# rkhosrowshahi/MO-VAE

Measured on NVIDIA B200. Metric: aggregation_GBps, higher is better.
Workload: dtype f32

## Files before the change

### mo-vae_b200/csrc/aggregate.cu

```cuda
#include "recombine_device.cuh"
#include "solve_device.cuh"

namespace movae {

int fill_solve_params(int k, const movae_solve_spec* spec, SolveParams* out);
int check_solve_vectors(const SolveParams& p, const float* d_vec, const float* d_aux);

constexpr int kAggThreads = 256;
static_assert(kAggThreads == kGramThreads && kAggThreads == kRecThreads && kAggThreads == kSolveThreads, "one CTA shape");

struct AggArgs {
    const float* J;
    int64_t P, ldJ;
    unsigned char* ws;
    const float* vec;
    const float* aux;
    float* out;
    int accumulate;
    float* w_out;
    double* diag_out;
    double* G_out;
};

template <int K>
__device__ __forceinline__ void aggregate_solve_phase(const SolveParams& sp, const P2PArgs& px, const float* vec, const float* aux,
                                                      float* w_out, double* diag_out, double* G_out, const double* partials,
                                                      unsigned int* ticket, unsigned int* ready, unsigned int ready0,
                                                      unsigned long long* stamps, unsigned long long t_start) {
    __shared__ SolveSmem S;
    __shared__ double Gs[K * K];
    __shared__ unsigned long long seq_s;
    __shared__ int failed_s;
    const int tid = threadIdx.x;
    const unsigned long long t_in = global_timer_ns();
    gram_combine_partials<K>(partials, Gs);
    if (tid == 0) { *ticket = 0u; failed_s = 0; stamps[4] = global_timer_ns(); }
    if (px.world > 0) {
        XchgBuffer* own = px.peers[px.rank];
        if (tid == 0) seq_s = own->step + 1;
        __syncthreads();
        const unsigned long long seq = seq_s;
        const int par = (int)(seq & 1ull);
        if (tid < K * K) {
            const double v = Gs[tid];
            for (int r = 0; r < px.world; ++r) st_relaxed_sys_f64(&px.peers[r]->slots[par][px.rank][tid], v);
        }
        __threadfence_system();
        __syncthreads();
        if (tid < px.world) st_release_sys_u64(&px.peers[tid]->flags[par][px.rank], seq);
        if (tid == 0) own->step = seq;
        if (tid < px.world && !wait_flag_sys(&own->flags[par][tid], seq, kExchangeTimeoutNs)) failed_s = 1;
        __syncthreads();
        if (tid < K * K) {
            double g = 0.0;
            for (int r = 0; r < px.world; ++r) g += ld_relaxed_sys_f64(&own->slots[par][r][tid]);
            Gs[tid] = g;
        }
        __syncthreads();
    }
    if (tid == 0) stamps[5] = global_timer_ns();
    if (tid < MK * MK) {
        const int i = tid / MK, j = tid % MK;
        S.G[i][j] = (i < K && j < K) ? Gs[i * K + j] : 0.0;
    }
    if (G_out && tid < K * K) G_out[tid] = Gs[tid];
    __syncthreads();
    solve_block<K>(sp, S, vec, aux, failed_s != 0, tid);
    if (tid < K) {
        w_out[tid] = S.w[tid];
        if (sp.comfort) w_out[K + tid] = S.w2[tid];
    }
    __syncthreads();
    if (tid == 0) {
        stamps[0] = t_start;
        stamps[1] = t_in;
        stamps[2] = global_timer_ns();
        __threadfence();
        st_release_gpu_u32(ready, ready0 + 1u);
    }
    solve_diagnostics(sp, S, tid);
    __syncthreads();
    if (tid < MOVAE_DIAG_DOUBLES && diag_out) diag_out[tid] = S.dg[tid];
}

__device__ __forceinline__ void aggregate_wait_ready(const unsigned int* ready, unsigned int ready0) {
    if (threadIdx.x == 0) {
        const unsigned long long t0 = global_timer_ns();
        while (ld_acquire_gpu_u32(ready) == ready0) {
            __nanosleep(40);
            if (global_timer_ns() - t0 > 2ull * kExchangeTimeoutNs) break;
        }
    }
    __syncthreads();
}

template <int K, int U1, int U2, bool VEC, int MINB>
__global__ void __launch_bounds__(kAggThreads, MINB)
aggregate_kernel(AggArgs a, SolveParams sp, P2PArgs px) {
    constexpr int NACC = GramAcc<K>::N;
    const int tid = threadIdx.x;
    unsigned int* ticket = reinterpret_cast<unsigned int*>(a.ws);
    unsigned int* done = reinterpret_cast<unsigned int*>(a.ws + 4);
    unsigned int* ready = reinterpret_cast<unsigned int*>(a.ws + 128);
    unsigned long long* stamps = reinterpret_cast<unsigned long long*>(a.ws + 192);
    double* partials = reinterpret_cast<double*>(a.ws + kGramHeaderBytes);

    __shared__ unsigned int ready0;
    __shared__ unsigned long long t_start;
    __shared__ double red[kGramThreads / 32][NACC];
    __shared__ int is_last;
    if (tid == 0) {
        ready0 = ld_acquire_gpu_u32(ready);
        t_start = global_timer_ns();
    }

    double acc64[NACC];
#pragma unroll
    for (int i = 0; i < NACC; ++i) acc64[i] = 0.0;
    gram_stream_tiles<K, U1, VEC>(a.J, a.P, a.ldJ, acc64);
    const bool last = gram_cta_partial_and_ticket<K>(acc64, partials, ticket, red, &is_last);

    if (last) aggregate_solve_phase<K>(sp, px, a.vec, a.aux, a.w_out, a.diag_out, a.G_out, partials, ticket, ready, ready0, stamps, t_start);
    if (a.out == nullptr) return;

    recombine_tiles<K, U2, VEC>(a.J, a.P, a.ldJ, a.w_out, a.out, a.accumulate, [&] {
        if (!last) aggregate_wait_ready(ready, ready0);
    });
    __syncthreads();
    if (tid == 0) {
        if (atomicAdd(done, 1u) == gridDim.x - 1) {
            stamps[3] = global_timer_ns();
            *done = 0u;
        }
    }
}

template <int K, int U1, int U2, bool VEC, int MINB>
static int launch_aggregate(const AggArgs& a, const SolveParams& sp, const P2PArgs& px, cudaStream_t st) {
    auto kern = aggregate_kernel<K, U1, U2, VEC, MINB>;
    static thread_local int occ_dev = -1, occ = 0;
    int dev = 0;
    MOVAE_CUDA_TRY(cudaGetDevice(&dev));
    if (occ_dev != dev) {
        MOVAE_CUDA_TRY(cudaOccupancyMaxActiveBlocksPerMultiprocessor(&occ, kern, kAggThreads, 0));
        if (occ < 1) occ = 1;
        occ_dev = dev;
    }
    const int sms = sm_count();
    MOVAE_REQUIRE(sms > 0, MOVAE_ERR_CUDA, "CUDA device query failed (no GPU?)");
    const int64_t n_items = a.P / (VEC ? 4 : 1);
    const int64_t tile_items = (int64_t)kAggThreads * (U1 > U2 ? U1 : U2);
    int64_t n_tiles = (n_items + tile_items - 1) / tile_items;
    if (n_tiles < 1) n_tiles = 1;
    int64_t grid = (int64_t)sms * occ;
    if (grid > n_tiles) grid = n_tiles;
    if (grid > kGramMaxBlocks) grid = kGramMaxBlocks;
    AggArgs a_ = a;
    SolveParams sp_ = sp;
    P2PArgs px_ = px;
    void* params[] = {&a_, &sp_, &px_};
    MOVAE_CUDA_TRY(cudaLaunchCooperativeKernel(reinterpret_cast<const void*>(kern), dim3((unsigned)grid), dim3(kAggThreads), params, 0, st));
    return MOVAE_OK;
}

template <int K>
static int dispatch_aggregate(const AggArgs& a, const SolveParams& sp, const P2PArgs& px, cudaStream_t st) {
    const bool vec = (reinterpret_cast<uintptr_t>(a.J) % 16 == 0) && (a.out == nullptr || reinterpret_cast<uintptr_t>(a.out) % 16 == 0) &&
                     (a.ldJ % 4 == 0 || K == 1);
    if (vec) {
        if constexpr (K <= 2) return launch_aggregate<K, 8, 4, true, 2>(a, sp, px, st);
        else if constexpr (K == 3) return launch_aggregate<K, 4, 4, true, 2>(a, sp, px, st);
        else if constexpr (K == 4) return launch_aggregate<K, 4, 2, true, 2>(a, sp, px, st);
        else return launch_aggregate<K, 2, 2, true, 1>(a, sp, px, st);
    } else {
        if constexpr (K <= 4) return launch_aggregate<K, 8, 8, false, 2>(a, sp, px, st);
        else return launch_aggregate<K, 4, 4, false, 1>(a, sp, px, st);
    }
}

struct SegArgs {
    movae_jac_segments segs;
    unsigned char* ws;
    const float* vec;
    const float* aux;
    float* out;
    int accumulate;
    float* w_out;
    double* diag_out;
    double* G_out;
};

template <int K, int U, int MINB>
__global__ void __launch_bounds__(kAggThreads, MINB)
aggregate_seg_kernel(const __grid_constant__ SegArgs a, SolveParams sp, P2PArgs px) {
    constexpr int NACC = GramAcc<K>::N;
    constexpr int kTile = kAggThreads * U;
    const int tid = threadIdx.x;
    unsigned int* ticket = reinterpret_cast<unsigned int*>(a.ws);
    unsigned int* done = reinterpret_cast<unsigned int*>(a.ws + 4);
    unsigned int* ready = reinterpret_cast<unsigned int*>(a.ws + 128);
    unsigned long long* stamps = reinterpret_cast<unsigned long long*>(a.ws + 192);
    double* partials = reinterpret_cast<double*>(a.ws + kGramHeaderBytes);
    const int n_seg = a.segs.n_segments;

    __shared__ unsigned int ready0;
    __shared__ unsigned long long t_start;
    __shared__ double red[kGramThreads / 32][NACC];
    __shared__ int is_last;
    __shared__ int tile_start[MOVAE_MAX_SEGMENTS + 1];
    if (tid == 0) {
        ready0 = ld_acquire_gpu_u32(ready);
        t_start = global_timer_ns();
        int acc = 0;
        for (int s = 0; s < n_seg; ++s) {
            tile_start[s] = acc;
            acc += (int)(((a.segs.n[s] >> 2) + kTile - 1) / kTile);
        }
        tile_start[n_seg] = acc;
    }
    __syncthreads();
    const int n_tiles = tile_start[n_seg];
    auto segment_of = [&](int v) { int s = 0; while (v >= tile_start[s + 1]) ++s; return s; };

    double acc64[NACC];
#pragma unroll
    for (int i = 0; i < NACC; ++i) acc64[i] = 0.0;
    for (int v = blockIdx.x; v < n_tiles; v += gridDim.x) {
        const int s = segment_of(v);
        const int64_t n_items = a.segs.n[s] >> 2;
        const int64_t base = (int64_t)(v - tile_start[s]) * kTile + tid;
        float4 x[K][U];
#pragma unroll
        for (int i = 0; i < K; ++i) {
            const float4* row = reinterpret_cast<const float4*>(a.segs.rows[s][i]);
#pragma unroll
            for (int u = 0; u < U; ++u) {
                const int64_t idx = base + u * kAggThreads;
                x[i][u] = idx < n_items ? ld_stream_f4(row + idx) : make_float4(0.f, 0.f, 0.f, 0.f);
            }
        }
        float acc[NACC];
#pragma unroll
        for (int q = 0; q < NACC; ++q) acc[q] = 0.f;
#pragma unroll
        for (int u = 0; u < U; ++u) {
            float c[K];
#pragma unroll
            for (int i = 0; i < K; ++i) c[i] = x[i][u].x;
            gram_fma<K>(acc, c);
#pragma unroll
            for (int i = 0; i < K; ++i) c[i] = x[i][u].y;
            gram_fma<K>(acc, c);
#pragma unroll
            for (int i = 0; i < K; ++i) c[i] = x[i][u].z;
            gram_fma<K>(acc, c);
#pragma unroll
            for (int i = 0; i < K; ++i) c[i] = x[i][u].w;
            gram_fma<K>(acc, c);
        }
#pragma unroll
        for (int q = 0; q < NACC; ++q) acc64[q] += (double)acc[q];
    }
    if (blockIdx.x == 0 && tid < 4 * n_seg) {
        const int s = tid >> 2, e = tid & 3;
        const int64_t c0 = a.segs.n[s] & ~(int64_t)3;
        if (c0 + e < a.segs.n[s]) {
            float c[K];
            float acc[NACC];
#pragma unroll
            for (int q = 0; q < NACC; ++q) acc[q] = 0.f;
#pragma unroll
            for (int i = 0; i < K; ++i) c[i] = a.segs.rows[s][i][c0 + e];
            gram_fma<K>(acc, c);
#pragma unroll
            for (int q = 0; q < NACC; ++q) acc64[q] += (double)acc[q];
        }
    }
    const bool last = gram_cta_partial_and_ticket<K>(acc64, partials, ticket, red, &is_last);

    if (last) aggregate_solve_phase<K>(sp, px, a.vec, a.aux, a.w_out, a.diag_out, a.G_out, partials, ticket, ready, ready0, stamps, t_start);
    if (a.out == nullptr) return;

    float w[K];
    bool have_w = false;
    for (int v = n_tiles - 1 - (int)blockIdx.x; v >= 0; v -= gridDim.x) {
        const int s = segment_of(v);
        const int64_t n_items = a.segs.n[s] >> 2;
        const int64_t base = (int64_t)(v - tile_start[s]) * kTile + tid;
        float4 x[K][U];
#pragma unroll
        for (int i = 0; i < K; ++i) {
            const float4* row = reinterpret_cast<const float4*>(a.segs.rows[s][i]);
#pragma unroll
            for (int u = 0; u < U; ++u) {
                const int64_t idx = base + u * kAggThreads;
                x[i][u] = idx < n_items ? ld_stream_f4(row + idx) : make_float4(0.f, 0.f, 0.f, 0.f);
            }
        }
        if (!have_w) {
            if (!last) aggregate_wait_ready(ready, ready0);
#pragma unroll
            for (int i = 0; i < K; ++i) w[i] = __ldcg(a.w_out + i);
            have_w = true;
        }
        float4* dst = reinterpret_cast<float4*>(a.out + a.segs.out_off[s]);
#pragma unroll
        for (int u = 0; u < U; ++u) {
            const int64_t idx = base + u * kAggThreads;
            if (idx >= n_items) continue;
            float4 o;
            o.x = w[0] * x[0][u].x; o.y = w[0] * x[0][u].y; o.z = w[0] * x[0][u].z; o.w = w[0] * x[0][u].w;
#pragma unroll
            for (int i = 1; i < K; ++i) {
                o.x = fmaf(w[i], x[i][u].x, o.x); o.y = fmaf(w[i], x[i][u].y, o.y);
                o.z = fmaf(w[i], x[i][u].z, o.z); o.w = fmaf(w[i], x[i][u].w, o.w);
            }
            if (a.accumulate) {
                const float4 old = dst[idx];
                o.x += old.x; o.y += old.y; o.z += old.z; o.w += old.w;
            }
            st_stream_f4(dst + idx, o);
        }
    }
    if (!have_w) {
        if (!last) aggregate_wait_ready(ready, ready0);
#pragma unroll
        for (int i = 0; i < K; ++i) w[i] = __ldcg(a.w_out + i);
    }
    if (blockIdx.x == 0 && tid < 4 * n_seg) {
        const int s = tid >> 2, e = tid & 3;
        const int64_t c = (a.segs.n[s] & ~(int64_t)3) + e;
        if (c < a.segs.n[s]) {
            float o = w[0] * a.segs.rows[s][0][c];
#pragma unroll
            for (int i = 1; i < K; ++i) o = fmaf(w[i], a.segs.rows[s][i][c], o);
            float* dst = a.out + a.segs.out_off[s] + c;
            *dst = a.accumulate ? *dst + o : o;
        }
    }
    __syncthreads();
    if (tid == 0) {
        if (atomicAdd(done, 1u) == gridDim.x - 1) {
            stamps[3] = global_timer_ns();
            *done = 0u;
        }
    }
}

template <int K, int U, int MINB>
static int launch_aggregate_seg(const SegArgs& a, const SolveParams& sp, const P2PArgs& px, cudaStream_t st) {
    auto kern = aggregate_seg_kernel<K, U, MINB>;
    static thread_local int occ_dev = -1, occ = 0;
    int dev = 0;
    MOVAE_CUDA_TRY(cudaGetDevice(&dev));
    if (occ_dev != dev) {
        MOVAE_CUDA_TRY(cudaOccupancyMaxActiveBlocksPerMultiprocessor(&occ, kern, kAggThreads, 0));
        if (occ < 1) occ = 1;
        occ_dev = dev;
    }
    const int sms = sm_count();
    MOVAE_REQUIRE(sms > 0, MOVAE_ERR_CUDA, "CUDA device query failed (no GPU?)");
    int64_t n_tiles = 0;
    for (int s = 0; s < a.segs.n_segments; ++s) n_tiles += ((a.segs.n[s] >> 2) + kAggThreads * U - 1) / (kAggThreads * U);
    if (n_tiles < 1) n_tiles = 1;
    int64_t grid = (int64_t)sms * occ;
    if (grid > n_tiles) grid = n_tiles;
    if (grid > kGramMaxBlocks) grid = kGramMaxBlocks;
    SegArgs a_ = a;
    SolveParams sp_ = sp;
    P2PArgs px_ = px;
    void* params[] = {&a_, &sp_, &px_};
    MOVAE_CUDA_TRY(cudaLaunchCooperativeKernel(reinterpret_cast<const void*>(kern), dim3((unsigned)grid), dim3(kAggThreads), params, 0, st));
    return MOVAE_OK;
}

}

extern "C" {

int movae_aggregate_f32(const float* d_J, int k, int64_t P, int64_t ldJ, const movae_solve_spec* spec, const float* d_vec,
                        const float* d_aux, float* d_grad, int accumulate, float* d_w, double* d_diag, double* d_G, void* d_ws,
                        size_t ws_bytes, const movae_p2p_ctx* ctx, void* stream) {
    using namespace movae;
    SolveParams sp;
    int rc = fill_solve_params(k, spec, &sp);
    if (rc != MOVAE_OK) return rc;
    rc = check_solve_vectors(sp, d_vec, d_aux);
    if (rc != MOVAE_OK) return rc;
    MOVAE_REQUIRE(P >= 0 && ldJ >= P, MOVAE_ERR_INVALID, "aggregate: need 0 <= P <= ldJ (P=%lld ldJ=%lld)", (long long)P, (long long)ldJ);
    MOVAE_REQUIRE(d_w != nullptr && (d_J != nullptr || P == 0), MOVAE_ERR_INVALID, "aggregate: null pointer");
    MOVAE_REQUIRE(d_ws != nullptr && ws_bytes >= movae_gram_workspace_bytes(k), MOVAE_ERR_WORKSPACE,
                  "aggregate: workspace too small (%zu < %zu)", ws_bytes, movae_gram_workspace_bytes(k));
    MOVAE_REQUIRE(reinterpret_cast<uintptr_t>(d_ws) % 8 == 0, MOVAE_ERR_WORKSPACE, "aggregate: workspace must be 8-byte aligned");
    P2PArgs px = p2p_disabled();
    if (ctx != nullptr) {
        rc = make_p2p_args(ctx, &px);
        if (rc != MOVAE_OK) return rc;
    }
    AggArgs a;
    a.J = d_J;
    a.P = P;
    a.ldJ = ldJ;
    a.ws = static_cast<unsigned char*>(d_ws);
    a.vec = d_vec;
    a.aux = d_aux;
    a.out = d_grad;
    a.accumulate = accumulate;
    a.w_out = d_w;
    a.diag_out = d_diag;
    a.G_out = d_G;
    cudaStream_t st = static_cast<cudaStream_t>(stream);
    switch (k) {
        case 1: return dispatch_aggregate<1>(a, sp, px, st);
        case 2: return dispatch_aggregate<2>(a, sp, px, st);
        case 3: return dispatch_aggregate<3>(a, sp, px, st);
        case 4: return dispatch_aggregate<4>(a, sp, px, st);
        case 5: return dispatch_aggregate<5>(a, sp, px, st);
        case 6: return dispatch_aggregate<6>(a, sp, px, st);
        case 7: return dispatch_aggregate<7>(a, sp, px, st);
        default: return dispatch_aggregate<8>(a, sp, px, st);
    }
}

int movae_aggregate_segments_f32(const movae_jac_segments* segs, const movae_solve_spec* spec, const float* d_vec,
                                 const float* d_aux, float* d_grad, int accumulate, float* d_w, double* d_diag, double* d_G,
                                 void* d_ws, size_t ws_bytes, const movae_p2p_ctx* ctx, void* stream) {
    using namespace movae;
    MOVAE_REQUIRE(segs != nullptr, MOVAE_ERR_INVALID, "aggregate_segments: null segment table");
    const int k = segs->k;
    SolveParams sp;
    int rc = fill_solve_params(k, spec, &sp);
    if (rc != MOVAE_OK) return rc;
    rc = check_solve_vectors(sp, d_vec, d_aux);
    if (rc != MOVAE_OK) return rc;
    MOVAE_REQUIRE(segs->n_segments >= 1 && segs->n_segments <= MOVAE_MAX_SEGMENTS, MOVAE_ERR_UNSUPPORTED,
                  "aggregate_segments: %d segments outside 1..%d", segs->n_segments, MOVAE_MAX_SEGMENTS);
    MOVAE_REQUIRE(d_w != nullptr, MOVAE_ERR_INVALID, "aggregate_segments: null pointer");
    MOVAE_REQUIRE(d_grad == nullptr || reinterpret_cast<uintptr_t>(d_grad) % 16 == 0, MOVAE_ERR_INVALID,
                  "aggregate_segments: the gradient buffer must be 16-byte aligned");
    for (int s = 0; s < segs->n_segments; ++s) {
        MOVAE_REQUIRE(segs->n[s] >= 0 && segs->out_off[s] >= 0 && segs->out_off[s] % 4 == 0, MOVAE_ERR_INVALID,
                      "aggregate_segments: segment %d needs n >= 0 and an output offset that is a multiple of 4", s);
        for (int i = 0; i < k; ++i)
            MOVAE_REQUIRE(segs->rows[s][i] != nullptr && reinterpret_cast<uintptr_t>(segs->rows[s][i]) % 16 == 0, MOVAE_ERR_INVALID,
                          "aggregate_segments: row %d of segment %d must be a 16-byte aligned device pointer", i, s);
    }
    MOVAE_REQUIRE(d_ws != nullptr && ws_bytes >= movae_gram_workspace_bytes(k), MOVAE_ERR_WORKSPACE,
                  "aggregate_segments: workspace too small (%zu < %zu)", ws_bytes, movae_gram_workspace_bytes(k));
    P2PArgs px = p2p_disabled();
    if (ctx != nullptr) {
        rc = make_p2p_args(ctx, &px);
        if (rc != MOVAE_OK) return rc;
    }
    SegArgs a;
    a.segs = *segs;
    a.ws = static_cast<unsigned char*>(d_ws);
    a.vec = d_vec;
    a.aux = d_aux;
    a.out = d_grad;
    a.accumulate = accumulate;
    a.w_out = d_w;
    a.diag_out = d_diag;
    a.G_out = d_G;
    cudaStream_t st = static_cast<cudaStream_t>(stream);
    switch (k) {
        case 1: return launch_aggregate_seg<1, 4, 2>(a, sp, px, st);
        case 2: return launch_aggregate_seg<2, 4, 2>(a, sp, px, st);
        case 3: return launch_aggregate_seg<3, 4, 2>(a, sp, px, st);
        case 4: return launch_aggregate_seg<4, 2, 2>(a, sp, px, st);
        case 5: return launch_aggregate_seg<5, 2, 1>(a, sp, px, st);
        case 6: return launch_aggregate_seg<6, 2, 1>(a, sp, px, st);
        case 7: return launch_aggregate_seg<7, 2, 1>(a, sp, px, st);
        default: return launch_aggregate_seg<8, 2, 1>(a, sp, px, st);
    }
}

int movae_aggregate_timestamps(const void* d_ws, uint64_t h_stamps[6], void* stream) {
    using namespace movae;
    MOVAE_REQUIRE(d_ws != nullptr && h_stamps != nullptr, MOVAE_ERR_INVALID, "aggregate_timestamps: null pointer");
    cudaStream_t st = static_cast<cudaStream_t>(stream);
    MOVAE_CUDA_TRY(cudaMemcpyAsync(h_stamps, static_cast<const unsigned char*>(d_ws) + 192, 6 * sizeof(uint64_t), cudaMemcpyDeviceToHost, st));
    MOVAE_CUDA_TRY(cudaStreamSynchronize(st));
    return MOVAE_OK;
}

}
```

### mo-vae_b200/csrc/common.cuh

```cuda
#pragma once
#include <cuda_runtime.h>
#include <stdint.h>
#include <stdio.h>
#include <string.h>

#include "../../include/movae_b200.h"

namespace movae {

void set_error(const char* fmt, ...);
int fail_cuda(cudaError_t e, const char* what);
int sm_count();

#define MOVAE_CUDA_TRY(expr)                                        \
    do {                                                            \
        cudaError_t _e = (expr);                                    \
        if (_e != cudaSuccess) return ::movae::fail_cuda(_e, #expr); \
    } while (0)

#define MOVAE_REQUIRE(cond, code, ...)          \
    do {                                        \
        if (!(cond)) {                          \
            ::movae::set_error(__VA_ARGS__);    \
            return (code);                      \
        }                                       \
    } while (0)

__device__ __forceinline__ float4 ld_stream_f4(const float4* p) {
    float4 v;
    asm volatile("ld.global.nc.L1::no_allocate.v4.f32 {%0,%1,%2,%3}, [%4];"
                 : "=f"(v.x), "=f"(v.y), "=f"(v.z), "=f"(v.w)
                 : "l"(p));
    return v;
}
__device__ __forceinline__ float ld_stream_f1(const float* p) {
    float v;
    asm volatile("ld.global.nc.L1::no_allocate.f32 %0, [%1];" : "=f"(v) : "l"(p));
    return v;
}
__device__ __forceinline__ void st_stream_f4(float4* p, float4 v) {
    asm volatile("st.global.cs.v4.f32 [%0], {%1,%2,%3,%4};" ::"l"(p), "f"(v.x), "f"(v.y), "f"(v.z), "f"(v.w)
                 : "memory");
}

struct XchgBuffer {
    double slots[2][MOVAE_MAX_WORLD][MOVAE_MAX_K * MOVAE_MAX_K];
    unsigned long long flags[2][MOVAE_MAX_WORLD];
    unsigned long long bar_flags[MOVAE_MAX_WORLD];
    unsigned long long step;
    unsigned long long bar_epoch;
};
struct P2PArgs {
    int rank, world;
    XchgBuffer* peers[MOVAE_MAX_WORLD];
};
__host__ __device__ inline P2PArgs p2p_disabled() {
    P2PArgs a;
    a.rank = 0;
    a.world = 0;
    for (int i = 0; i < MOVAE_MAX_WORLD; ++i) a.peers[i] = nullptr;
    return a;
}
int make_p2p_args(const movae_p2p_ctx* ctx, P2PArgs* out);

__device__ __forceinline__ void st_release_sys_u64(unsigned long long* p, unsigned long long v) {
    asm volatile("st.release.sys.global.u64 [%0], %1;" ::"l"(p), "l"(v) : "memory");
}
__device__ __forceinline__ unsigned long long ld_acquire_sys_u64(const unsigned long long* p) {
    unsigned long long v;
    asm volatile("ld.acquire.sys.global.u64 %0, [%1];" : "=l"(v) : "l"(p) : "memory");
    return v;
}
__device__ __forceinline__ double ld_relaxed_sys_f64(const double* p) {
    double v;
    asm volatile("ld.relaxed.sys.global.f64 %0, [%1];" : "=d"(v) : "l"(p) : "memory");
    return v;
}

__device__ __forceinline__ void st_relaxed_sys_f64(double* p, double v) {
    asm volatile("st.relaxed.sys.global.f64 [%0], %1;" ::"l"(p), "d"(v) : "memory");
}
__device__ __forceinline__ void st_release_gpu_u32(unsigned int* p, unsigned int v) {
    asm volatile("st.release.gpu.global.u32 [%0], %1;" ::"l"(p), "r"(v) : "memory");
}
__device__ __forceinline__ unsigned int ld_acquire_gpu_u32(const unsigned int* p) {
    unsigned int v;
    asm volatile("ld.acquire.gpu.global.u32 %0, [%1];" : "=r"(v) : "l"(p) : "memory");
    return v;
}
__device__ __forceinline__ unsigned long long global_timer_ns() {
    unsigned long long t;
    asm volatile("mov.u64 %0, %%globaltimer;" : "=l"(t));
    return t;
}
__device__ __forceinline__ bool wait_flag_sys(const unsigned long long* flag, unsigned long long want,
                                              unsigned long long timeout_ns) {
    if (ld_acquire_sys_u64(flag) >= want) return true;
    const unsigned long long t0 = global_timer_ns();
    while (ld_acquire_sys_u64(flag) < want) {
        if (global_timer_ns() - t0 > timeout_ns) return false;
    }
    return true;
}
constexpr unsigned long long kExchangeTimeoutNs = 20ull * 1000ull * 1000ull * 1000ull;

__device__ __forceinline__ double warp_sum(double v) {
#pragma unroll
    for (int o = 16; o > 0; o >>= 1) v += __shfl_xor_sync(0xffffffffu, v, o);
    return v;
}

}
```

### mo-vae_b200/csrc/gram_device.cuh

```cuda
#pragma once
#include "common.cuh"

namespace movae {

constexpr int kGramThreads = 256;
constexpr int kGramMaxBlocks = 2048;
constexpr int kGramHeaderBytes = 256;
constexpr int kGramChain = 64;

template <int K>
struct GramAcc {
    static constexpr int N = K * (K + 1) / 2;
};

template <int K>
__device__ __forceinline__ void gram_fma(float (&acc)[GramAcc<K>::N], const float (&x)[K]) {
    int a = 0;
#pragma unroll
    for (int i = 0; i < K; ++i)
#pragma unroll
        for (int j = i; j < K; ++j) { acc[a] = fmaf(x[i], x[j], acc[a]); ++a; }
}

struct RRSchedule {
    int64_t rounds;
    int64_t rem_lo, rem_hi;
};
__device__ __forceinline__ RRSchedule rr_schedule(int64_t n_items, int64_t tile_items, int64_t b, int64_t g) {
    RRSchedule s;
    s.rounds = (n_items / tile_items) / g;
    const int64_t r0 = s.rounds * g * tile_items;
    const int64_t m = (((n_items - r0) + g - 1) / g + 7) & ~(int64_t)7;
    s.rem_lo = r0 + b * m < n_items ? r0 + b * m : n_items;
    s.rem_hi = s.rem_lo + m < n_items ? s.rem_lo + m : n_items;
    return s;
}

template <int K, int U, bool VEC>
__device__ __forceinline__ void gram_tile(const float* __restrict__ J, int64_t ldJ, int64_t t0, int64_t hi, bool full,
                                          float (&acc)[GramAcc<K>::N]) {
    const int64_t base = t0 + threadIdx.x;
    if constexpr (VEC) {
        float4 v[K][U];
        if (full) {
#pragma unroll
            for (int i = 0; i < K; ++i)
#pragma unroll
                for (int u = 0; u < U; ++u)
                    v[i][u] = ld_stream_f4(reinterpret_cast<const float4*>(J + i * ldJ) + base + u * kGramThreads);
        } else {
#pragma unroll
            for (int i = 0; i < K; ++i)
#pragma unroll
                for (int u = 0; u < U; ++u) {
                    const int64_t idx = base + u * kGramThreads;
                    v[i][u] = idx < hi ? ld_stream_f4(reinterpret_cast<const float4*>(J + i * ldJ) + idx)
                                       : make_float4(0.f, 0.f, 0.f, 0.f);
                }
        }
#pragma unroll
        for (int u = 0; u < U; ++u) {
            float x[K];
#pragma unroll
            for (int i = 0; i < K; ++i) x[i] = v[i][u].x;
            gram_fma<K>(acc, x);
#pragma unroll
            for (int i = 0; i < K; ++i) x[i] = v[i][u].y;
            gram_fma<K>(acc, x);
#pragma unroll
            for (int i = 0; i < K; ++i) x[i] = v[i][u].z;
            gram_fma<K>(acc, x);
#pragma unroll
            for (int i = 0; i < K; ++i) x[i] = v[i][u].w;
            gram_fma<K>(acc, x);
        }
    } else {
        float v[K][U];
#pragma unroll
        for (int i = 0; i < K; ++i)
#pragma unroll
            for (int u = 0; u < U; ++u) {
                const int64_t idx = base + u * kGramThreads;
                v[i][u] = idx < hi ? ld_stream_f1(J + i * ldJ + idx) : 0.f;
            }
#pragma unroll
        for (int u = 0; u < U; ++u) {
            float x[K];
#pragma unroll
            for (int i = 0; i < K; ++i) x[i] = v[i][u];
            gram_fma<K>(acc, x);
        }
    }
}

template <int K, int U, bool VEC>
__device__ __forceinline__ void gram_stream_tiles(const float* __restrict__ J, int64_t P, int64_t ldJ,
                                                  double (&acc64)[GramAcc<K>::N]) {
    constexpr int NACC = GramAcc<K>::N;
    constexpr int W = VEC ? 4 : 1;
    constexpr int FLUSH = kGramChain / (W * U) > 0 ? kGramChain / (W * U) : 1;
    const int tid = threadIdx.x;
    const int64_t n_items = P / W;
    constexpr int64_t tile_items = (int64_t)kGramThreads * U;
    const RRSchedule sch = rr_schedule(n_items, tile_items, blockIdx.x, gridDim.x);

    int64_t r = 0;
    while (r < sch.rounds) {
        float acc[NACC];
#pragma unroll
        for (int a = 0; a < NACC; ++a) acc[a] = 0.f;
#pragma unroll 1
        for (int f = 0; f < FLUSH && r < sch.rounds; ++f, ++r) {
            const int64_t t0 = (r * gridDim.x + blockIdx.x) * tile_items;
            gram_tile<K, U, VEC>(J, ldJ, t0, t0 + tile_items, true, acc);
        }
#pragma unroll
        for (int a = 0; a < NACC; ++a) acc64[a] += (double)acc[a];
    }
    if (sch.rem_hi > sch.rem_lo) {
        float acc[NACC];
#pragma unroll
        for (int a = 0; a < NACC; ++a) acc[a] = 0.f;
        gram_tile<K, U, VEC>(J, ldJ, sch.rem_lo, sch.rem_hi, false, acc);
#pragma unroll
        for (int a = 0; a < NACC; ++a) acc64[a] += (double)acc[a];
    }

    if (VEC && blockIdx.x == 0 && tid < (int)(P - n_items * W)) {
        float x[K];
        float acc[NACC];
#pragma unroll
        for (int a = 0; a < NACC; ++a) acc[a] = 0.f;
#pragma unroll
        for (int i = 0; i < K; ++i) x[i] = J[i * ldJ + n_items * W + tid];
        gram_fma<K>(acc, x);
#pragma unroll
        for (int a = 0; a < NACC; ++a) acc64[a] += (double)acc[a];
    }
}

template <int K>
__device__ __forceinline__ bool gram_cta_partial_and_ticket(const double (&acc64)[GramAcc<K>::N], double* __restrict__ partials,
                                                            unsigned int* __restrict__ counter,
                                                            double (*red)[GramAcc<K>::N], int* is_last_smem) {
    constexpr int NACC = GramAcc<K>::N;
    const int tid = threadIdx.x, warp = tid >> 5, lane = tid & 31;
#pragma unroll
    for (int a = 0; a < NACC; ++a) {
        const double s = warp_sum(acc64[a]);
        if (lane == 0) red[warp][a] = s;
    }
    __syncthreads();
    if (tid < NACC) {
        double s = 0.0;
#pragma unroll
        for (int w = 0; w < kGramThreads / 32; ++w) s += red[w][tid];
        partials[(int64_t)blockIdx.x * NACC + tid] = s;
    }
    __threadfence();
    __syncthreads();
    if (tid == 0) *is_last_smem = (atomicAdd(counter, 1u) == gridDim.x - 1);
    __syncthreads();
    return *is_last_smem != 0;
}

template <int K>
__device__ __forceinline__ void gram_combine_partials(const double* __restrict__ partials, double* __restrict__ Gs) {
    constexpr int NACC = GramAcc<K>::N;
    const int tid = threadIdx.x, warp = tid >> 5, lane = tid & 31;
    __threadfence();
    for (int a = warp; a < NACC; a += kGramThreads / 32) {
        double s0 = 0.0, s1 = 0.0, s2 = 0.0, s3 = 0.0;
        const int g = (int)gridDim.x;
        for (int b = lane; b < g; b += 128) {
            const double v0 = __ldcg(&partials[(int64_t)b * NACC + a]);
            const double v1 = b + 32 < g ? __ldcg(&partials[(int64_t)(b + 32) * NACC + a]) : 0.0;
            const double v2 = b + 64 < g ? __ldcg(&partials[(int64_t)(b + 64) * NACC + a]) : 0.0;
            const double v3 = b + 96 < g ? __ldcg(&partials[(int64_t)(b + 96) * NACC + a]) : 0.0;
            s0 += v0; s1 += v1; s2 += v2; s3 += v3;
        }
        double s = (s0 + s1) + (s2 + s3);
        s = warp_sum(s);
        if (lane == 0) {
            int i = 0, rem = a;
            while (rem >= K - i) { rem -= K - i; ++i; }
            const int j = i + rem;
            Gs[i * K + j] = s;
            Gs[j * K + i] = s;
        }
    }
    __syncthreads();
}

}
```

### mo-vae_b200/csrc/recombine_device.cuh

```cuda
#pragma once
#include <type_traits>

#include "gram_device.cuh"

namespace movae {

constexpr int kRecThreads = 256;

template <int K, int U, bool VEC>
struct RecTile {
    using T = typename std::conditional<VEC, float4, float>::type;
    T v[K][U];
};

template <int K, int U, bool VEC>
__device__ __forceinline__ void rec_load_tile(RecTile<K, U, VEC>& r, const float* __restrict__ J, int64_t ldJ, int64_t base,
                                              int64_t lo, int64_t hi, bool full) {
#pragma unroll
    for (int i = 0; i < K; ++i)
#pragma unroll
        for (int u = 0; u < U; ++u) {
            const int64_t idx = base + u * kRecThreads;
            if constexpr (VEC)
                r.v[i][u] = (full || (idx >= lo && idx < hi)) ? ld_stream_f4(reinterpret_cast<const float4*>(J + i * ldJ) + idx)
                                                    : make_float4(0.f, 0.f, 0.f, 0.f);
            else
                r.v[i][u] = (full || (idx >= lo && idx < hi)) ? ld_stream_f1(J + i * ldJ + idx) : 0.f;
        }
}

template <int K, int U, bool VEC>
__device__ __forceinline__ void rec_store_tile(const RecTile<K, U, VEC>& r, const float (&w)[K], float* __restrict__ out,
                                               int64_t base, int64_t lo, int64_t hi, bool full, int accumulate) {
#pragma unroll
    for (int u = 0; u < U; ++u) {
        const int64_t idx = base + u * kRecThreads;
        if (!full && (idx < lo || idx >= hi)) continue;
        if constexpr (VEC) {
            float4 o;
            o.x = w[0] * r.v[0][u].x; o.y = w[0] * r.v[0][u].y; o.z = w[0] * r.v[0][u].z; o.w = w[0] * r.v[0][u].w;
#pragma unroll
            for (int i = 1; i < K; ++i) {
                o.x = fmaf(w[i], r.v[i][u].x, o.x); o.y = fmaf(w[i], r.v[i][u].y, o.y);
                o.z = fmaf(w[i], r.v[i][u].z, o.z); o.w = fmaf(w[i], r.v[i][u].w, o.w);
            }
            float4* dst = reinterpret_cast<float4*>(out) + idx;
            if (accumulate) {
                const float4 old = *dst;
                o.x += old.x; o.y += old.y; o.z += old.z; o.w += old.w;
            }
            st_stream_f4(dst, o);
        } else {
            float o = w[0] * r.v[0][u];
#pragma unroll
            for (int i = 1; i < K; ++i) o = fmaf(w[i], r.v[i][u], o);
            if (accumulate) o += out[idx];
            out[idx] = o;
        }
    }
}

template <int K, int U, bool VEC, class Ready>
__device__ __forceinline__ void recombine_tiles(const float* __restrict__ J, int64_t P, int64_t ldJ, const float* w_dev,
                                                float* __restrict__ out, int accumulate, Ready ready) {
    constexpr int W = VEC ? 4 : 1;
    const int tid = threadIdx.x;
    const int64_t n_items = P / W;
    constexpr int64_t tile_items = (int64_t)kRecThreads * U;
    const RRSchedule sch = rr_schedule(n_items, tile_items, blockIdx.x, gridDim.x);
    const bool has_rem = sch.rem_hi > sch.rem_lo;
    const int64_t n_steps = sch.rounds + (has_rem ? 1 : 0);
    auto t0_of = [&](int64_t i) -> int64_t {
        if (has_rem) { if (i == 0) return sch.rem_lo; --i; }
        return ((sch.rounds - 1 - i) * gridDim.x + blockIdx.x) * tile_items;
    };
    auto hi_of = [&](int64_t i, int64_t t0) -> int64_t { return (has_rem && i == 0) ? sch.rem_hi : t0 + tile_items; };
    auto full_of = [&](int64_t i) -> bool { return !(has_rem && i == 0); };

    RecTile<K, U, VEC> ra, rb;
    int64_t i = 0;
    int64_t ta = 0, tb = 0;
    if (n_steps > 0) { ta = t0_of(0); rec_load_tile<K, U, VEC>(ra, J, ldJ, ta + tid, ta, hi_of(0, ta), full_of(0)); }
    ready();
    float w[K];
#pragma unroll
    for (int q = 0; q < K; ++q) w[q] = __ldcg(w_dev + q);
    while (i < n_steps) {
        const bool has_b = i + 1 < n_steps;
        if (has_b) { tb = t0_of(i + 1); rec_load_tile<K, U, VEC>(rb, J, ldJ, tb + tid, tb, hi_of(i + 1, tb), full_of(i + 1)); }
        rec_store_tile<K, U, VEC>(ra, w, out, ta + tid, ta, hi_of(i, ta), full_of(i), accumulate);
        if (!has_b) break;
        if (i + 2 < n_steps) { ta = t0_of(i + 2); rec_load_tile<K, U, VEC>(ra, J, ldJ, ta + tid, ta, hi_of(i + 2, ta), full_of(i + 2)); }
        rec_store_tile<K, U, VEC>(rb, w, out, tb + tid, tb, hi_of(i + 1, tb), full_of(i + 1), accumulate);
        i += 2;
    }
    if (VEC && blockIdx.x == 0 && tid < (int)(P - n_items * W)) {
        const int64_t c = n_items * W + tid;
        float o = w[0] * J[c];
#pragma unroll
        for (int q = 1; q < K; ++q) o = fmaf(w[q], J[q * ldJ + c], o);
        if (accumulate) o += out[c];
        out[c] = o;
    }
}

}
```

Before: 6364.

## Pin tail of J in L2 with evict_last for reuse by recombine pass

The gram pass now loads the last rounds of J, sized to about two thirds of L2, with an evict_last cache policy. The recombine pass walks tiles in reverse order, so it can hit those lines in L2 instead of re-reading DRAM, and it demotes each consumed line back to evict_normal. This cuts DRAM traffic for the second read of J. It adds createpolicy and applypriority instructions, and the pinned data can crowd out other cached lines.

```diff
diff --git a/mo-vae_b200/csrc/aggregate.cu b/mo-vae_b200/csrc/aggregate.cu
--- a/mo-vae_b200/csrc/aggregate.cu
+++ b/mo-vae_b200/csrc/aggregate.cu
@@ -20,7 +20,10 @@
     float* w_out;
     double* diag_out;
     double* G_out;
+    int64_t keep_lo;
 };
+
+constexpr int64_t kL2KeepNum = 2, kL2KeepDen = 3;
 
 template <int K>
 __device__ __forceinline__ void aggregate_solve_phase(const SolveParams& sp, const P2PArgs& px, const float* vec, const float* aux,
@@ -117,7 +120,7 @@
     double acc64[NACC];
 #pragma unroll
     for (int i = 0; i < NACC; ++i) acc64[i] = 0.0;
-    gram_stream_tiles<K, U1, VEC>(a.J, a.P, a.ldJ, acc64);
+    gram_stream_tiles<K, U1, VEC>(a.J, a.P, a.ldJ, acc64, a.keep_lo);
     const bool last = gram_cta_partial_and_ticket<K>(acc64, partials, ticket, red, &is_last);
 
     if (last) aggregate_solve_phase<K>(sp, px, a.vec, a.aux, a.w_out, a.diag_out, a.G_out, partials, ticket, ready, ready0, stamps, t_start);
@@ -125,7 +128,7 @@
 
     recombine_tiles<K, U2, VEC>(a.J, a.P, a.ldJ, a.w_out, a.out, a.accumulate, [&] {
         if (!last) aggregate_wait_ready(ready, ready0);
-    });
+    }, a.keep_lo);
     __syncthreads();
     if (tid == 0) {
         if (atomicAdd(done, 1u) == gridDim.x - 1) {
@@ -138,12 +141,13 @@
 template <int K, int U1, int U2, bool VEC, int MINB>
 static int launch_aggregate(const AggArgs& a, const SolveParams& sp, const P2PArgs& px, cudaStream_t st) {
     auto kern = aggregate_kernel<K, U1, U2, VEC, MINB>;
-    static thread_local int occ_dev = -1, occ = 0;
+    static thread_local int occ_dev = -1, occ = 0, l2_bytes = 0;
     int dev = 0;
     MOVAE_CUDA_TRY(cudaGetDevice(&dev));
     if (occ_dev != dev) {
         MOVAE_CUDA_TRY(cudaOccupancyMaxActiveBlocksPerMultiprocessor(&occ, kern, kAggThreads, 0));
         if (occ < 1) occ = 1;
+        MOVAE_CUDA_TRY(cudaDeviceGetAttribute(&l2_bytes, cudaDevAttrL2CacheSize, dev));
         occ_dev = dev;
     }
     const int sms = sm_count();
@@ -156,6 +160,14 @@
     if (grid > n_tiles) grid = n_tiles;
     if (grid > kGramMaxBlocks) grid = kGramMaxBlocks;
     AggArgs a_ = a;
+    a_.keep_lo = INT64_MAX;
+    if (VEC && a.out != nullptr) {
+        const int64_t rec_tile = (int64_t)kAggThreads * U2;
+        const int64_t round_bytes = grid * rec_tile * K * (int64_t)sizeof(float4);
+        const int64_t keep_rounds = (int64_t)l2_bytes * kL2KeepNum / kL2KeepDen / round_bytes;
+        const int64_t first = (a.P / 4 / rec_tile) / grid - keep_rounds;
+        a_.keep_lo = (first > 0 ? first : 0) * grid * rec_tile;
+    }
     SolveParams sp_ = sp;
     P2PArgs px_ = px;
     void* params[] = {&a_, &sp_, &px_};
diff --git a/mo-vae_b200/csrc/common.cuh b/mo-vae_b200/csrc/common.cuh
--- a/mo-vae_b200/csrc/common.cuh
+++ b/mo-vae_b200/csrc/common.cuh
@@ -38,6 +38,20 @@
     asm volatile("ld.global.nc.L1::no_allocate.f32 %0, [%1];" : "=f"(v) : "l"(p));
     return v;
 }
+__device__ __forceinline__ float4 ld_keep_f4(const float4* p) {
+    uint64_t pol;
+    asm volatile("createpolicy.fractional.L2::evict_last.b64 %0, 1.0;" : "=l"(pol));
+    float4 v;
+    asm volatile("ld.global.nc.L1::no_allocate.L2::cache_hint.v4.f32 {%0,%1,%2,%3}, [%4], %5;"
+                 : "=f"(v.x), "=f"(v.y), "=f"(v.z), "=f"(v.w)
+                 : "l"(p), "l"(pol));
+    return v;
+}
+__device__ __forceinline__ void l2_demote_line(const void* p) {
+    asm volatile("applypriority.global.L2::evict_normal [%0], 128;" ::"l"(reinterpret_cast<uintptr_t>(p) & ~(uintptr_t)127)
+                 : "memory");
+}
+
 __device__ __forceinline__ void st_stream_f4(float4* p, float4 v) {
     asm volatile("st.global.cs.v4.f32 [%0], {%1,%2,%3,%4};" ::"l"(p), "f"(v.x), "f"(v.y), "f"(v.z), "f"(v.w)
                  : "memory");
diff --git a/mo-vae_b200/csrc/gram_device.cuh b/mo-vae_b200/csrc/gram_device.cuh
--- a/mo-vae_b200/csrc/gram_device.cuh
+++ b/mo-vae_b200/csrc/gram_device.cuh
@@ -36,25 +36,27 @@
     return s;
 }
 
-template <int K, int U, bool VEC>
+template <int K, int U, bool VEC, bool KEEP = false>
 __device__ __forceinline__ void gram_tile(const float* __restrict__ J, int64_t ldJ, int64_t t0, int64_t hi, bool full,
                                           float (&acc)[GramAcc<K>::N]) {
+    static_assert(VEC || !KEEP, "evict_last loads are float4-path only");
     const int64_t base = t0 + threadIdx.x;
     if constexpr (VEC) {
+        auto ld = [](const float4* p) { if constexpr (KEEP) return ld_keep_f4(p); else return ld_stream_f4(p); };
         float4 v[K][U];
         if (full) {
 #pragma unroll
             for (int i = 0; i < K; ++i)
 #pragma unroll
                 for (int u = 0; u < U; ++u)
-                    v[i][u] = ld_stream_f4(reinterpret_cast<const float4*>(J + i * ldJ) + base + u * kGramThreads);
+                    v[i][u] = ld(reinterpret_cast<const float4*>(J + i * ldJ) + base + u * kGramThreads);
         } else {
 #pragma unroll
             for (int i = 0; i < K; ++i)
 #pragma unroll
                 for (int u = 0; u < U; ++u) {
                     const int64_t idx = base + u * kGramThreads;
-                    v[i][u] = idx < hi ? ld_stream_f4(reinterpret_cast<const float4*>(J + i * ldJ) + idx)
+                    v[i][u] = idx < hi ? ld(reinterpret_cast<const float4*>(J + i * ldJ) + idx)
                                        : make_float4(0.f, 0.f, 0.f, 0.f);
                 }
         }
@@ -95,7 +97,7 @@
 
 template <int K, int U, bool VEC>
 __device__ __forceinline__ void gram_stream_tiles(const float* __restrict__ J, int64_t P, int64_t ldJ,
-                                                  double (&acc64)[GramAcc<K>::N]) {
+                                                  double (&acc64)[GramAcc<K>::N], int64_t keep_lo = INT64_MAX) {
     constexpr int NACC = GramAcc<K>::N;
     constexpr int W = VEC ? 4 : 1;
     constexpr int FLUSH = kGramChain / (W * U) > 0 ? kGramChain / (W * U) : 1;
@@ -112,7 +114,8 @@
 #pragma unroll 1
         for (int f = 0; f < FLUSH && r < sch.rounds; ++f, ++r) {
             const int64_t t0 = (r * gridDim.x + blockIdx.x) * tile_items;
-            gram_tile<K, U, VEC>(J, ldJ, t0, t0 + tile_items, true, acc);
+            if (VEC && t0 + tile_items > keep_lo) gram_tile<K, U, VEC, VEC>(J, ldJ, t0, t0 + tile_items, true, acc);
+            else gram_tile<K, U, VEC>(J, ldJ, t0, t0 + tile_items, true, acc);
         }
 #pragma unroll
         for (int a = 0; a < NACC; ++a) acc64[a] += (double)acc[a];
@@ -121,7 +124,8 @@
         float acc[NACC];
 #pragma unroll
         for (int a = 0; a < NACC; ++a) acc[a] = 0.f;
-        gram_tile<K, U, VEC>(J, ldJ, sch.rem_lo, sch.rem_hi, false, acc);
+        if (VEC && sch.rem_hi > keep_lo) gram_tile<K, U, VEC, VEC>(J, ldJ, sch.rem_lo, sch.rem_hi, false, acc);
+        else gram_tile<K, U, VEC>(J, ldJ, sch.rem_lo, sch.rem_hi, false, acc);
 #pragma unroll
         for (int a = 0; a < NACC; ++a) acc64[a] += (double)acc[a];
     }
diff --git a/mo-vae_b200/csrc/recombine_device.cuh b/mo-vae_b200/csrc/recombine_device.cuh
--- a/mo-vae_b200/csrc/recombine_device.cuh
+++ b/mo-vae_b200/csrc/recombine_device.cuh
@@ -60,9 +60,22 @@
     }
 }
 
+template <int K, int U>
+__device__ __forceinline__ void rec_demote_tile(const float* __restrict__ J, int64_t ldJ, int64_t base, int64_t hi, bool full) {
+    if ((threadIdx.x & 7) != 0) return;
+#pragma unroll
+    for (int u = 0; u < U; ++u) {
+        const int64_t idx = base + u * kRecThreads;
+        if (!full && idx >= hi) continue;
+#pragma unroll
+        for (int i = 0; i < K; ++i) l2_demote_line(reinterpret_cast<const float4*>(J + i * ldJ) + idx);
+    }
+}
+
 template <int K, int U, bool VEC, class Ready>
 __device__ __forceinline__ void recombine_tiles(const float* __restrict__ J, int64_t P, int64_t ldJ, const float* w_dev,
-                                                float* __restrict__ out, int accumulate, Ready ready) {
+                                                float* __restrict__ out, int accumulate, Ready ready,
+                                                int64_t keep_lo = INT64_MAX) {
     constexpr int W = VEC ? 4 : 1;
     const int tid = threadIdx.x;
     const int64_t n_items = P / W;
@@ -89,9 +102,11 @@
         const bool has_b = i + 1 < n_steps;
         if (has_b) { tb = t0_of(i + 1); rec_load_tile<K, U, VEC>(rb, J, ldJ, tb + tid, tb, hi_of(i + 1, tb), full_of(i + 1)); }
         rec_store_tile<K, U, VEC>(ra, w, out, ta + tid, ta, hi_of(i, ta), full_of(i), accumulate);
+        if (VEC && hi_of(i, ta) > keep_lo) rec_demote_tile<K, U>(J, ldJ, ta + tid, hi_of(i, ta), full_of(i));
         if (!has_b) break;
         if (i + 2 < n_steps) { ta = t0_of(i + 2); rec_load_tile<K, U, VEC>(ra, J, ldJ, ta + tid, ta, hi_of(i + 2, ta), full_of(i + 2)); }
         rec_store_tile<K, U, VEC>(rb, w, out, tb + tid, tb, hi_of(i + 1, tb), full_of(i + 1), accumulate);
+        if (VEC && hi_of(i + 1, tb) > keep_lo) rec_demote_tile<K, U>(J, ldJ, tb + tid, hi_of(i + 1, tb), full_of(i + 1));
         i += 2;
     }
     if (VEC && blockIdx.x == 0 && tid < (int)(P - n_items * W)) {
```

Result: no change. 6342 (median of 6 runs) (-0.3%).
